# HpWang-whu/YOHO

Hardware: AMD Instinct MI355X
Metric: keypoints/sec (5000 kp x60 rot desc+YOHO-O) (higher is better)
Workload: dtype fp16x2 split (2^-22-accurate products, fp32 accumulate); 1 GPU

## Files before the change

### yoho_amd/csrc/gemmf2.hip

```cpp
#include <hip/hip_runtime.h>
#include <cstdlib>
#include <cstring>
#include "common.h"
#include "gemmf.h"

namespace yoho {

constexpr int F2_BUF = 24576;
constexpr int F2_LDS = 3 * F2_BUF;
constexpr int F3_BUF = 32768;
constexpr int F3_LDS = 3 * F3_BUF;

struct Frags2 {
    uintx4 ah[4], al[4], bh[2], bl[2];
};

template <int LO, int R>
__device__ __forceinline__ void read_frag2(const char* pa, const char* pb, Frags2& f) {
    if constexpr (R < 4) f.al[R] = *reinterpret_cast<const uintx4*>(pa + 8192 + R * 512);
    else if constexpr (R < 6) f.bh[R - 4] = *reinterpret_cast<const uintx4*>(pb + (R - 4) * 512);
    else if constexpr (R < 10) f.ah[R - 6] = *reinterpret_cast<const uintx4*>(pa + (R - 6) * 512);
    else f.bl[R - 10] = *reinterpret_cast<const uintx4*>(pb + LO + (R - 10) * 512);
}
template <int LO>
__device__ __forceinline__ void read_frags2(const char* pa, const char* pb, Frags2& f) {
    sfor<0, 12>([&](auto rc) { read_frag2<LO, decltype(rc)::value>(pa, pb, f); });
}

struct Dma2 {
    static constexpr int NP = 6, LO = 4096;
    int la, lb, w;
    __device__ __forceinline__ Dma2(int w_, int lane) : la(w_ * 1024 + lane * 16), lb((w_ >> 1) * 4096 + (w_ & 1) * 1024 + lane * 16), w(w_) {}
    template <int U>
    __device__ __forceinline__ void piece(const char* srcA, const char* srcB, char* buf) const {
        if constexpr (U < 4) {
            constexpr int plane = U >> 1, kg = U & 1;
            __builtin_amdgcn_global_load_lds((gptr_t)(srcA + plane * 16384 + kg * 4096 + la), (lptr_t)(buf + plane * 8192 + kg * 4096 + w * 1024), 16, 0, 0);
        } else {
            constexpr int plane = U - 4;
            __builtin_amdgcn_global_load_lds((gptr_t)(srcB + plane * 16384 + lb), (lptr_t)(buf + 16384 + plane * 4096 + (w >> 1) * 2048 + (w & 1) * 1024), 16, 0, 0);
        }
    }
};
struct Dma3 {
    static constexpr int NP = 4, LO = 8192;
    int la, ldst;
    __device__ __forceinline__ Dma3(int w8, int lane) : la(w8 * 1024 + lane * 16), ldst(w8 * 1024) {}
    template <int U>
    __device__ __forceinline__ void piece(const char* srcA, const char* srcB, char* buf) const {
        constexpr int plane = U & 1;
        if constexpr (U < 2) __builtin_amdgcn_global_load_lds((gptr_t)(srcA + plane * 16384 + la), (lptr_t)(buf + plane * 8192 + ldst), 16, 0, 0);
        else __builtin_amdgcn_global_load_lds((gptr_t)(srcB + plane * 16384 + la), (lptr_t)(buf + 16384 + plane * 8192 + ldst), 16, 0, 0);
    }
};
template <typename Dma>
__device__ __forceinline__ void dma_step(const Dma& dm, const char* srcA, const char* srcB, char* buf) {
    sfor<0, Dma::NP>([&](auto uc) { dm.template piece<decltype(uc)::value>(srcA, srcB, buf); });
}

template <bool DMA, typename Dma>
__device__ __forceinline__ void step2(const Dma& dm, const Frags2& f, floatx16 (&acc)[4][2], const char* ra, const char* rb, Frags2& nf,
                                      const char* srcA, const char* srcB, char* dmabuf) {
    sfor<0, 8>([&](auto gc) {
        constexpr int g = decltype(gc)::value;
        acc[g >> 1][g & 1] = mfma_h(f.al[g >> 1], f.bh[g & 1], acc[g >> 1][g & 1]);
        read_frag2<Dma::LO, g>(ra, rb, nf);
        __builtin_amdgcn_sched_barrier(0);
    });
    sfor<0, 8>([&](auto gc) {
        constexpr int g = decltype(gc)::value;
        acc[g >> 1][g & 1] = mfma_h(f.ah[g >> 1], f.bl[g & 1], acc[g >> 1][g & 1]);
        if constexpr (g < 4) read_frag2<Dma::LO, 8 + g>(ra, rb, nf);
        else if constexpr (DMA) dm.template piece<g - 4>(srcA, srcB, dmabuf);
        __builtin_amdgcn_sched_barrier(0);
    });
    sfor<0, 8>([&](auto gc) {
        constexpr int g = decltype(gc)::value;
        acc[g >> 1][g & 1] = mfma_h(f.ah[g >> 1], f.bh[g & 1], acc[g >> 1][g & 1]);
        if constexpr (DMA && 4 + g < Dma::NP) dm.template piece<4 + g>(srcA, srcB, dmabuf);
        __builtin_amdgcn_sched_barrier(0);
    });
}

__host__ __device__ inline bool fg2_map(const FGemmArgs& a, int xcd, int slot, bool contiguous, int& t, int& local, int& r) {
    int cnt[NIR_ORD], ru[NIR_ORD];
    for (int u = 0; u < NIR_ORD; ++u) {
        ru[u] = (xcd + a.rot[u]) & 7;
        cnt[u] = a.NT[u] > ru[u] ? ((a.NT[u] - 1 - ru[u]) / 8 + 1) * a.MT[u] * 2 : 0;
    }
    const int L = cnt[0], S = cnt[1] + cnt[2] + cnt[3] + cnt[4];
    int list, idx;
    if (contiguous) { list = slot < L ? 0 : 1; idx = slot < L ? slot : slot - L; }
    else {
        const int P = L < S ? L : S;
        if (slot < 2 * P) { list = slot & 1; idx = slot >> 1; }
        else { list = L > S ? 0 : 1; idx = P + (slot - 2 * P); }
    }
    if (list == 0) {
        if (idx >= L) return false;
        t = 0; local = idx; r = ru[0];
        return true;
    }
    for (int u = 1; u < NIR_ORD; ++u) {
        if (idx < cnt[u]) { t = u; local = idx; r = ru[u]; return true; }
        idx -= cnt[u];
    }
    return false;
}

__device__ __forceinline__ size_t step_off(int ks) { return (size_t)(ks >> 1) * FG_STAGE + (size_t)(ks & 1) * 8192; }

template <int BUF, typename Dma>
__device__ __forceinline__ void ring_prologue(int KT, Dma&& dma) {
    dma(0, 0);
    dma(1, BUF);
    if (KT > 2) dma(2, 2 * BUF);
}

template <int BUF, int INFLIGHT, typename F, typename Step>
__device__ __forceinline__ void ring_pipelined(char* smem, const char* Ag, const char* Bg, int KT, int lane_a, int lane_b, F& P, Step&& step) {
    F Q;
    asm volatile("s_waitcnt lgkmcnt(0)" ::: "memory");
    __builtin_amdgcn_s_barrier();
    __builtin_amdgcn_sched_barrier(0);
    int cur = 0, nxt = BUF;
    int s = 0;
    auto run = [&](auto dma, const F& f, F& nf) {
        if constexpr (decltype(dma)::value) {
            step(dma, f, nf, smem + nxt + lane_a, smem + nxt + lane_b, uniform_ptr(Ag + step_off(s + 3)), uniform_ptr(Bg + step_off(s + 3)), smem + cur);
            asm volatile("s_waitcnt vmcnt(%0) lgkmcnt(0)" ::"n"(INFLIGHT) : "memory");
        } else {
            step(dma, f, nf, smem + nxt + lane_a, smem + nxt + lane_b, nullptr, nullptr, nullptr);
            asm volatile("s_waitcnt vmcnt(0) lgkmcnt(0)" ::: "memory");
        }
        __builtin_amdgcn_s_barrier();
        __builtin_amdgcn_sched_barrier(0);
        cur = nxt; nxt = nxt == 2 * BUF ? 0 : nxt + BUF; ++s;
    };
    constexpr std::true_type dma;
    constexpr std::false_type nodma;
    while (s + 4 < KT) {
        run(dma, P, Q);
        run(dma, Q, P);
    }
    if (KT >= 4) {
        run(dma, P, Q);
        run(nodma, Q, P);
    }
    run(nodma, P, Q);
    step(nodma, Q, P, smem + cur + lane_a, smem + cur + lane_b, nullptr, nullptr, nullptr);
}

template <int BUF, typename Dma>
__device__ __forceinline__ void ring_pipelined_idle(int KT, Dma&& dma) {
    __builtin_amdgcn_s_barrier();
    for (int s = 0; s + 1 < KT; ++s) {
        if (s + 3 < KT) dma(s + 3, (s % 3) * BUF);
        asm volatile("s_waitcnt vmcnt(0)" ::: "memory");
        __builtin_amdgcn_s_barrier();
    }
}

__global__ __launch_bounds__(256, 2) void fgemm2_kernel(FGemmArgs a, int flags) {
    extern __shared__ __attribute__((aligned(16))) char smem[];
    const int tid = threadIdx.x, lane = tid & 63;
    const int w = __builtin_amdgcn_readfirstlane(tid >> 6);
    int t = 0, local = 0, r = 0;
    if (!fg2_map(a, blockIdx.x & 7, blockIdx.x >> 3, (flags & F2_MIX) == 0, t, local, r)) return;
    const int d = a.dim[t];
    const int MT = a.MT[t], KS = d * a.cin / 32, KT = 2 * KS;
    const int nh = local & 1, pair = local >> 1;
    const int cg = pair / MT, mtile = pair - cg * MT;
    const int ntile = r + 8 * cg;
    const char* Ag = a.A + a.a_off[t] + (size_t)mtile * KS * FG_STAGE;
    const char* Bg = a.B + a.b_off[t] + (size_t)ntile * KS * FG_STAGE + nh * 2048;
    const int wm = w >> 1, wn = w & 1;
    const Dma2 dm(w, lane);
    const int lane_a = (lane >> 5) * 4096 + (wm * 128 + (lane & 31)) * 16;
    const int lane_b = 16384 + (lane >> 5) * 2048 + (wn * 64 + (lane & 31)) * 16;

    floatx16 acc[4][2];
    zero_acc(acc);
    auto dma = [&](int st, int buf) { dma_step(dm, Ag + step_off(st), Bg + step_off(st), smem + buf); };
    ring_prologue<F2_BUF>(KT, dma);
    const int row0 = mtile * 256 + wm * 128, colbase = ntile * 256 + nh * 128 + wn * 64;
    const bool rows_live = row0 < d * a.cout;
    const int jidx = colbase / a.kppad, kp0 = colbase - jidx * a.kppad, qbase = a.qbase[t];
    if ((flags & EPI_RES) && rows_live) residual_start(acc, row0, kp0, jidx, d, qbase, a.res, a.descale, a.cout, a.nT32, lane);
    asm volatile("s_waitcnt vmcnt(0)" ::: "memory");
    __builtin_amdgcn_s_barrier();
    if (!rows_live) return ring_pipelined_idle<F2_BUF>(KT, dma);

    Frags2 P;
    read_frags2<Dma2::LO>(smem + lane_a, smem + lane_b, P);
    ring_pipelined<F2_BUF, 6>(smem, Ag, Bg, KT, lane_a, lane_b, P,
        [&](auto dmac, const Frags2& f, Frags2& nf, const char* ra, const char* rb, const char* srcA, const char* srcB, char* buf) {
            step2<decltype(dmac)::value>(dm, f, acc, ra, rb, nf, srcA, srcB, buf);
        });
    coef_epilogue(acc, row0, kp0, jidx, d, qbase, a.out, a.bias, a.descale, a.cout, a.nT32, a.rflag, lane, flags);
}

struct Wave3 {
    int wm, wn, nh, lane_a, lane_b;
    Dma3 dm;
    __device__ __forceinline__ Wave3(int w8, int lane) : wm((w8 & 3) >> 1), wn(w8 & 1), nh(w8 >> 2), dm(w8, lane) {
        lane_a = (lane >> 5) * 4096 + (wm * 128 + (lane & 31)) * 16;
        lane_b = 16384 + (lane >> 5) * 4096 + (nh * 128 + wn * 64 + (lane & 31)) * 16;
    }
};

__global__ __launch_bounds__(512, 2) void fgemm3_kernel(FGemmArgs a, int flags) {
    extern __shared__ __attribute__((aligned(16))) char smem[];
    const int tid = threadIdx.x, lane = tid & 63;
    const Wave3 wv(__builtin_amdgcn_readfirstlane(tid >> 6), lane);
    int t = 0, local = 0, r = 0;
    if (!fg3_map(a, blockIdx.x & 7, blockIdx.x >> 3, t, local, r)) return;
    const int d = a.dim[t];
    const int MT = a.MT[t], KS = d * a.cin / 32, KT = 2 * KS;
    const int cg = local / MT, mtile = local - cg * MT;
    const int ntile = r + 8 * cg;
    const char* Ag = a.A + a.a_off[t] + (size_t)mtile * KS * FG_STAGE;
    const char* Bg = a.B + a.b_off[t] + (size_t)ntile * KS * FG_STAGE;

    floatx16 acc[4][2];
    zero_acc(acc);
    auto dma = [&](int st, int buf) { dma_step(wv.dm, Ag + step_off(st), Bg + step_off(st), smem + buf); };
    ring_prologue<F3_BUF>(KT, dma);
    const int row0 = mtile * 256 + wv.wm * 128, colbase = ntile * 256 + wv.nh * 128 + wv.wn * 64;
    const bool rows_live = row0 < d * a.cout;
    const int jidx = colbase / a.kppad, kp0 = colbase - jidx * a.kppad, qbase = a.qbase[t];
    if ((flags & EPI_RES) && rows_live) residual_start(acc, row0, kp0, jidx, d, qbase, a.res, a.descale, a.cout, a.nT32, lane);
    asm volatile("s_waitcnt vmcnt(0)" ::: "memory");
    __builtin_amdgcn_s_barrier();
    if (!rows_live) return ring_pipelined_idle<F3_BUF>(KT, dma);

    Frags2 P;
    read_frags2<Dma3::LO>(smem + wv.lane_a, smem + wv.lane_b, P);
    ring_pipelined<F3_BUF, 4>(smem, Ag, Bg, KT, wv.lane_a, wv.lane_b, P,
        [&](auto dmac, const Frags2& f, Frags2& nf, const char* ra, const char* rb, const char* srcA, const char* srcB, char* buf) {
            step2<decltype(dmac)::value>(wv.dm, f, acc, ra, rb, nf, srcA, srcB, buf);
        });
    coef_epilogue(acc, row0, kp0, jidx, d, qbase, a.out, a.bias, a.descale, a.cout, a.nT32, a.rflag, lane, flags);
}

constexpr int F3K_BUF = 2 * FG_STAGE;
constexpr int F3K_LDS = 2 * F3K_BUF;

struct Dma3k {
    static constexpr int NP = 8;
    int la, ldst;
    __device__ __forceinline__ Dma3k(int w8, int lane) : la(w8 * 1024 + lane * 16), ldst(w8 * 1024) {}
    template <int U>
    __device__ __forceinline__ void piece(const char* srcA, const char* srcB, char* buf) const {
        constexpr int q = (U & 3) * 8192;
        if constexpr (U < 4) __builtin_amdgcn_global_load_lds((gptr_t)(srcA + q + la), (lptr_t)(buf + q + ldst), 16, 0, 0);
        else __builtin_amdgcn_global_load_lds((gptr_t)(srcB + q + la), (lptr_t)(buf + FG_STAGE + q + ldst), 16, 0, 0);
    }
};
struct FragsA32 { uintx4 al, ah; };
struct FragsB32 { uintx4 bh[4], bl[4]; };

template <int R>
__device__ __forceinline__ void read_open32(const char* pa, const char* pb, FragsA32& a0, FragsB32& b) {
    if constexpr (R == 0) a0.al = *reinterpret_cast<const uintx4*>(pa + 16384);
    else if constexpr (R < 5) b.bh[R - 1] = *reinterpret_cast<const uintx4*>(pb + (R - 1) * 256);
    else if constexpr (R == 5) a0.ah = *reinterpret_cast<const uintx4*>(pa);
    else b.bl[R - 6] = *reinterpret_cast<const uintx4*>(pb + 16384 + (R - 6) * 256);
}

template <bool DMA>
__device__ __forceinline__ void step32(const Dma3k& dm, floatx4 (&acc)[8][4], FragsA32 (&fa)[2], const FragsB32& b, FragsB32& nb, const char* pa,
                                       const char* npa, const char* npb, const char* srcA, const char* srcB, char* dmabuf) {
    sfor<0, 7>([&](auto ic) {
        constexpr int i = decltype(ic)::value;
        row_products32(acc[i], fa[i & 1].al, fa[i & 1].ah, b.bh, b.bl, [&](auto mc) {
            constexpr int m = decltype(mc)::value;
            if constexpr (m == 1) fa[(i + 1) & 1].al = *reinterpret_cast<const uintx4*>(pa + 16384 + (i + 1) * 256);
            if constexpr (m == 2) fa[(i + 1) & 1].ah = *reinterpret_cast<const uintx4*>(pa + (i + 1) * 256);
        });
    });
    asm volatile("s_waitcnt vmcnt(0) lgkmcnt(0)" ::: "memory");
    __builtin_amdgcn_s_barrier();
    __builtin_amdgcn_sched_barrier(0);
    row_products32(acc[7], fa[1].al, fa[1].ah, b.bh, b.bl, [&](auto mc) {
        constexpr int m = decltype(mc)::value;
        if constexpr (m < 5) {
            read_open32<2 * m>(npa, npb, fa[0], nb);
            read_open32<2 * m + 1>(npa, npb, fa[0], nb);
        }
        if constexpr (DMA && m >= 4) dm.template piece<m - 4>(srcA, srcB, dmabuf);
    });
}

__global__ __launch_bounds__(512, 2) void fgemm3k_kernel(FGemmArgs a, int flags) {
    extern __shared__ __attribute__((aligned(16))) char smem[];
    const int tid = threadIdx.x, lane = tid & 63;
    const int w8 = __builtin_amdgcn_readfirstlane(tid >> 6);
    int t = 0, local = 0, r = 0;
    if (!fg3_map(a, blockIdx.x & 7, blockIdx.x >> 3, t, local, r)) return;
    const int d = a.dim[t];
    const int MT = a.MT[t], KS = d * a.cin / 32;
    const int cg = local / MT, mtile = local - cg * MT;
    const int ntile = r + 8 * cg;
    const char* Ag = a.A + a.a_off[t] + (size_t)mtile * KS * FG_STAGE;
    const char* Bg = a.B + a.b_off[t] + (size_t)ntile * KS * FG_STAGE;
    const int wm = (w8 & 3) >> 1, wn = w8 & 1, nh = w8 >> 2;
    const Dma3k dm(w8, lane);
    const int lane_a = (lane >> 4) * 4096 + (wm * 128 + (lane & 15)) * 16;
    const int lane_b = FG_STAGE + (lane >> 4) * 4096 + (nh * 128 + wn * 64 + (lane & 15)) * 16;

    floatx4 acc[8][4];
    zero_acc(acc);
    auto dma = [&](int st, int buf) {
        const char* sa = uniform_ptr(Ag + (size_t)st * FG_STAGE);
        const char* sb = uniform_ptr(Bg + (size_t)st * FG_STAGE);
        sfor<0, Dma3k::NP>([&](auto uc) { dm.template piece<decltype(uc)::value>(sa, sb, smem + buf); });
    };
    dma(0, 0);
    if (KS > 1) dma(1, F3K_BUF);
    const int row0 = mtile * 256 + wm * 128, colbase = ntile * 256 + nh * 128 + wn * 64;
    const bool rows_live = row0 < d * a.cout;
    const int jidx = colbase / a.kppad, kp0 = colbase - jidx * a.kppad, qbase = a.qbase[t];
    if ((flags & EPI_RES) && rows_live) residual_start(acc, row0, kp0, jidx, d, qbase, a.res, a.descale, a.cout, a.nT32, lane);
    asm volatile("s_waitcnt vmcnt(0)" ::: "memory");
    __builtin_amdgcn_s_barrier();
    if (!rows_live) {
        for (int s = 0; s < KS; ++s) {
            asm volatile("s_waitcnt vmcnt(0)" ::: "memory");
            __builtin_amdgcn_s_barrier();
            if (s + 2 < KS) dma(s + 2, (s & 1) * F3K_BUF);
        }
        asm volatile("s_waitcnt vmcnt(0)" ::: "memory");
        return;
    }

    FragsA32 fa[2];
    FragsB32 P, Q;
    sfor<0, 10>([&](auto rc) { read_open32<decltype(rc)::value>(smem + lane_a, smem + lane_b, fa[0], P); });
    int s = 0, cur = 0;
    auto run = [&](auto dmac, const FragsB32& b, FragsB32& nb) {
        const int nxt = cur ^ F3K_BUF;
        if constexpr (decltype(dmac)::value)
            step32<true>(dm, acc, fa, b, nb, smem + cur + lane_a, smem + nxt + lane_a, smem + nxt + lane_b, uniform_ptr(Ag + (size_t)(s + 2) * FG_STAGE),
                         uniform_ptr(Bg + (size_t)(s + 2) * FG_STAGE), smem + cur);
        else
            step32<false>(dm, acc, fa, b, nb, smem + cur + lane_a, smem + nxt + lane_a, smem + nxt + lane_b, nullptr, nullptr, nullptr);
        cur = nxt; ++s;
    };
    constexpr std::true_type dmay;
    constexpr std::false_type dman;
    while (s + 2 < KS) {
        run(dmay, P, Q);
        run(dmay, Q, P);
    }
    run(dman, P, Q);
    run(dman, Q, P);
    coef_epilogue(acc, row0, kp0, jidx, d, qbase, a.out, a.bias, a.descale, a.cout, a.nT32, a.rflag, lane, flags);
}

constexpr int F2K_BUF = FG_STAGE + FG_STAGE / 2;
constexpr int F2K_LDS = 2 * F2K_BUF;

__global__ __launch_bounds__(256, 1) void fgemm2k_kernel(FGemmArgs a, int flags) {
    extern __shared__ __attribute__((aligned(16))) char smem[];
    const int tid = threadIdx.x, lane = tid & 63;
    const int w = __builtin_amdgcn_readfirstlane(tid >> 6);
    int t = 0, local = 0, r = 0;
    if (!fg2_map(a, blockIdx.x & 7, blockIdx.x >> 3, (flags & F2_MIX) == 0, t, local, r)) return;
    const int d = a.dim[t];
    const int MT = a.MT[t], KS = d * a.cin / 32;
    const int nh = local & 1, pair = local >> 1;
    const int cg = pair / MT, mtile = pair - cg * MT;
    const int ntile = r + 8 * cg;
    const char* Ag = a.A + a.a_off[t] + (size_t)mtile * KS * FG_STAGE;
    const char* Bg = a.B + a.b_off[t] + (size_t)ntile * KS * FG_STAGE + nh * 2048;
    const int wm = w >> 1, wn = w & 1;
    const int lane_a = (lane >> 4) * 4096 + (wm * 128 + (lane & 15)) * 16;
    const int lane_b = FG_STAGE + (lane >> 4) * 2048 + (wn * 64 + (lane & 15)) * 16;

    floatx4 acc[8][4];
    zero_acc(acc);
    auto dma = [&](int st, int buf) {
        const char* sa = uniform_ptr(Ag + (size_t)st * FG_STAGE) + lane * 16;
        const char* sb = uniform_ptr(Bg + (size_t)st * FG_STAGE) + lane * 16;
#pragma unroll
        for (int k = 0; k < 8; ++k) __builtin_amdgcn_global_load_lds((gptr_t)(sa + (k * 4 + w) * 1024), (lptr_t)(smem + buf + (k * 4 + w) * 1024), 16, 0, 0);
#pragma unroll
        for (int k = 0; k < 4; ++k) {
            const int pb = w * 4 + k, u = pb >> 1, part = pb & 1;
            __builtin_amdgcn_global_load_lds((gptr_t)(sb + u * 4096 + part * 1024), (lptr_t)(smem + buf + FG_STAGE + u * 2048 + part * 1024), 16, 0, 0);
        }
    };
    dma(0, 0);
    if (KS > 1) dma(1, F2K_BUF);
    const int row0 = mtile * 256 + wm * 128, colbase = ntile * 256 + nh * 128 + wn * 64;
    const bool rows_live = row0 < d * a.cout;
    const int jidx = colbase / a.kppad, kp0 = colbase - jidx * a.kppad, qbase = a.qbase[t];
    if ((flags & EPI_RES) && rows_live) residual_start(acc, row0, kp0, jidx, d, qbase, a.res, a.descale, a.cout, a.nT32, lane);
    asm volatile("s_waitcnt vmcnt(0)" ::: "memory");
    __builtin_amdgcn_s_barrier();
    for (int s = 0; s < KS; ++s) {
        const int cur = (s & 1) * F2K_BUF;
        if (rows_live) stage32_plain<FG_STAGE / 4>(acc, smem + cur + lane_a, smem + cur + lane_b);
        asm volatile("s_waitcnt vmcnt(0) lgkmcnt(0)" ::: "memory");
        __builtin_amdgcn_s_barrier();
        __builtin_amdgcn_sched_barrier(0);
        if (s + 2 < KS) dma(s + 2, cur);
    }
    if (rows_live) coef_epilogue(acc, row0, kp0, jidx, d, qbase, a.out, a.bias, a.descale, a.cout, a.nT32, a.rflag, lane, flags);
}

typedef int intx8 __attribute__((ext_vector_type(8)));
typedef short shortx2 __attribute__((ext_vector_type(2)));
typedef _Float16 halfx2 __attribute__((ext_vector_type(2)));
struct Frags8 {
    intx8 a[4], b[2];
};
struct C8Scales {
    float ah = 4.f, al = 4.f / 2048.f, bh = 1.f, bl = 1.f;
    int mfma_b = 127;
    C8Scales() = default;
    __device__ __forceinline__ explicit C8Scales(const unsigned* amax) {
        const unsigned amax_bits = __builtin_amdgcn_readfirstlane(*amax);
        int kexp = (int)(amax_bits >> 23) - 127 - 7;
        kexp = kexp < -60 ? -60 : (kexp > 9 ? 9 : kexp);
        bh = __uint_as_float((unsigned)(kexp + 127) << 23); bl = __uint_as_float((unsigned)(kexp - 11 + 127) << 23);
        mfma_b = 127 + kexp;
    }
};
struct Int2 { int x, y; };
__device__ __forceinline__ Int2 frag_to_fp8(uintx4 f, float scale) {
    union { unsigned u; halfx2 h; } p0, p1, p2, p3;
    p0.u = f[0]; p1.u = f[1]; p2.u = f[2]; p3.u = f[3];
    shortx2 r = {0, 0}, q = {0, 0};
    r = __builtin_amdgcn_cvt_scalef32_pk_fp8_f16(r, p0.h, scale, false);
    r = __builtin_amdgcn_cvt_scalef32_pk_fp8_f16(r, p1.h, scale, true);
    q = __builtin_amdgcn_cvt_scalef32_pk_fp8_f16(q, p2.h, scale, false);
    q = __builtin_amdgcn_cvt_scalef32_pk_fp8_f16(q, p3.h, scale, true);
    Int2 o;
    __builtin_memcpy(&o.x, &r, 4);
    __builtin_memcpy(&o.y, &q, 4);
    return o;
}

template <int PAR>
__device__ __forceinline__ void step3c(const Frags2& f, floatx16 (&acc)[4][2], Frags8& c8, const C8Scales& sc) {
#pragma unroll
    for (int i = 0; i < 4; ++i)
#pragma unroll
        for (int j = 0; j < 2; ++j) acc[i][j] = mfma_h(f.ah[i], f.bh[j], acc[i][j]);
#pragma unroll
    for (int i = 0; i < 4; ++i)
#pragma unroll
        for (int e = 0; e < 4; ++e) c8.a[i][4 * PAR + e] = (int)f.al[i][e];
#pragma unroll
    for (int j = 0; j < 2; ++j) {
        const Int2 l = frag_to_fp8(f.bl[j], sc.bl), h = frag_to_fp8(f.bh[j], sc.bh);
        c8.b[j][4 * PAR] = l.x; c8.b[j][4 * PAR + 1] = l.y; c8.b[j][4 * PAR + 2] = h.x; c8.b[j][4 * PAR + 3] = h.y;
    }
    if constexpr (PAR == 1) {
#pragma unroll
        for (int i = 0; i < 4; ++i)
#pragma unroll
            for (int j = 0; j < 2; ++j)
                acc[i][j] = __builtin_amdgcn_mfma_scale_f32_32x32x64_f8f6f4(c8.a[i], c8.b[j], acc[i][j], 0, 0, 0, 127 + 2 - 11, 0, sc.mfma_b);
    }
}

template <bool FP8, typename BSrc>
__device__ __forceinline__ void ring_plain(floatx16 (&acc)[4][2], char* smem, const Wave3& wv, const char* Ag, BSrc&& bsrc, int KT, bool rows_live,
                                           const C8Scales& sc) {
    Frags8 c8;
    if constexpr (FP8) {
#pragma unroll
        for (int i = 0; i < 4; ++i)
#pragma unroll
            for (int e = 0; e < 8; ++e) c8.a[i][e] = 0;
#pragma unroll
        for (int j = 0; j < 2; ++j)
#pragma unroll
            for (int e = 0; e < 8; ++e) c8.b[j][e] = 0;
    }
    int cur = 0, stg = 2 * F3_BUF;
    int s = 0;
    auto stage = [&] {
        const int s2 = s + 2 < KT ? s + 2 : KT - 1;
        dma_step(wv.dm, uniform_ptr(Ag + step_off(s2)), uniform_ptr(bsrc(s2)), smem + stg);
    };
    auto rotate = [&] { stg = cur; cur = cur == 2 * F3_BUF ? 0 : cur + F3_BUF; ++s; };
    auto one_step = [&](auto parity) {
        asm volatile("s_waitcnt vmcnt(4) lgkmcnt(0)" ::: "memory");
        __builtin_amdgcn_s_barrier();
        __builtin_amdgcn_sched_barrier(0);
        stage();
        Frags2 f;
        read_frags2<Dma3::LO>(smem + cur + wv.lane_a, smem + cur + wv.lane_b, f);
        if constexpr (FP8) step3c<decltype(parity)::value>(f, acc, c8, sc);
        else {
#pragma unroll
            for (int i = 0; i < 4; ++i)
#pragma unroll
                for (int j = 0; j < 2; ++j) acc[i][j] = mfma_h(f.al[i], f.bh[j], acc[i][j]);
#pragma unroll
            for (int i = 0; i < 4; ++i)
#pragma unroll
                for (int j = 0; j < 2; ++j) acc[i][j] = mfma_h(f.ah[i], f.bl[j], acc[i][j]);
#pragma unroll
            for (int i = 0; i < 4; ++i)
#pragma unroll
                for (int j = 0; j < 2; ++j) acc[i][j] = mfma_h(f.ah[i], f.bh[j], acc[i][j]);
        }
        rotate();
    };
    if (rows_live) {
        for (int it = 0; it < KT; it += 2) {
            one_step(std::integral_constant<int, 0>{});
            one_step(std::integral_constant<int, 1>{});
        }
    } else {
        for (int it = 0; it < KT; ++it) {
            asm volatile("s_waitcnt vmcnt(4) lgkmcnt(0)" ::: "memory");
            __builtin_amdgcn_s_barrier();
            stage();
            rotate();
        }
    }
    asm volatile("s_waitcnt vmcnt(0)" ::: "memory");
}

__global__ __launch_bounds__(512, 2) void fgemm3c_kernel(FGemmArgs a, int flags) {
    extern __shared__ __attribute__((aligned(16))) char smem[];
    const int tid = threadIdx.x, lane = tid & 63;
    const Wave3 wv(__builtin_amdgcn_readfirstlane(tid >> 6), lane);
    int t = 0, local = 0, r = 0;
    if (!fg3_map(a, blockIdx.x & 7, blockIdx.x >> 3, t, local, r)) return;
    const int d = a.dim[t];
    const int MT = a.MT[t], KS = d * a.cin / 32, KT = 2 * KS;
    const int cg = local / MT, mtile = local - cg * MT;
    const int ntile = r + 8 * cg;
    const char* Ag = a.A + a.a_off[t] + (size_t)mtile * KS * FG_STAGE;
    const char* Bg = a.B + a.b_off[t] + (size_t)ntile * KS * FG_STAGE;

    floatx16 acc[4][2];
    zero_acc(acc);
    const C8Scales sc(a.amax);
    dma_step(wv.dm, Ag, Bg, smem);
    dma_step(wv.dm, Ag + step_off(1), Bg + step_off(1), smem + F3_BUF);
    const int row0 = mtile * 256 + wv.wm * 128, colbase = ntile * 256 + wv.nh * 128 + wv.wn * 64;
    const bool rows_live = row0 < d * a.cout;
    const int jidx = colbase / a.kppad, kp0 = colbase - jidx * a.kppad, qbase = a.qbase[t];
    if ((flags & EPI_RES) && rows_live) residual_start(acc, row0, kp0, jidx, d, qbase, a.res, a.descale, a.cout, a.nT32, lane);
    asm volatile("s_waitcnt vmcnt(0)" ::: "memory");
    __builtin_amdgcn_s_barrier();

    ring_plain<true>(acc, smem, wv, Ag, [&](int s) { return Bg + step_off(s); }, KT, rows_live, sc);
    if (rows_live) coef_epilogue(acc, row0, kp0, jidx, d, qbase, a.out, a.bias, a.descale, a.cout, a.nT32, a.rflag, lane, flags);
}

struct CGemmArgs {
    const char* A;
    const char* B;
    const float* bias;
    const float* bn_s;
    const float* bn_t;
    char* out;
    int NTm, MT, KSt, ntap, nj, nslot, c8out, nT32, nTiles16;
    float descale;
    int* rflag;
    const unsigned* amax;
    unsigned char slot[13 * 13];
    unsigned char outg[16];
};

__device__ __forceinline__ void cg_split_pair(float x0, float x1, unsigned& hi, unsigned& lo) {
    typedef float f2 __attribute__((ext_vector_type(2)));
    f2 x;
    x.x = x0; x.y = x1;
    const halfx2 h = __builtin_convertvector(x, halfx2);
    const f2 r = x - __builtin_convertvector(h, f2);
    const halfx2 l = __builtin_convertvector(r, halfx2);
    __builtin_memcpy(&hi, &h, 4);
    __builtin_memcpy(&lo, &l, 4);
}

template <bool FP8>
__global__ __launch_bounds__(512, 2) void cgemm_kernel(CGemmArgs a) {
    extern __shared__ __attribute__((aligned(16))) char smem[];
    __shared__ int tapoff[16];
    const int tid = threadIdx.x, lane = tid & 63;
    const Wave3 wv(__builtin_amdgcn_readfirstlane(tid >> 6), lane);
    const int xcd = blockIdx.x & 7, slot_ = blockIdx.x >> 3;
    const int ct = xcd + 8 * (slot_ / a.MT), mtile = slot_ % a.MT;
    if (ct >= a.nj * a.NTm) return;
    const int j = ct / a.NTm, mt = ct - j * a.NTm;
    const int SPT = 2 * a.KSt;
    const int KT = a.ntap * SPT;
    if (tid < 16) tapoff[tid] = tid < a.ntap ? (int)a.slot[j * 13 + tid] : 0;
    const char* Ag = a.A + (size_t)mtile * (KT / 2) * FG_STAGE;
    const char* Bt = a.B + (size_t)mt * a.nslot * a.KSt * FG_STAGE;
    __syncthreads();
    auto bsrc = [&](int s) -> const char* {
        const int tap = s / SPT, within = s - tap * SPT;
        const int sl = __builtin_amdgcn_readfirstlane(tapoff[tap]);
        return Bt + (size_t)sl * a.KSt * FG_STAGE + step_off(within);
    };

    floatx16 acc[4][2];
    zero_acc(acc);
    C8Scales sc;
    if constexpr (FP8) sc = C8Scales(a.amax);
    dma_step(wv.dm, Ag, uniform_ptr(bsrc(0)), smem);
    dma_step(wv.dm, Ag + step_off(1), uniform_ptr(bsrc(1)), smem + F3_BUF);
    asm volatile("s_waitcnt vmcnt(0)" ::: "memory");
    __builtin_amdgcn_s_barrier();

    ring_plain<FP8>(acc, smem, wv, Ag, bsrc, KT, true, sc);

    const int half = lane >> 5, c32 = lane & 31;
    const int g = a.outg[j];
    unsigned top = 0u;
#pragma unroll
    for (int bi = 0; bi < 2; ++bi) {
        const int m = mt * 256 + wv.nh * 128 + wv.wn * 64 + bi * 32 + c32;
        if ((m >> 5) >= a.nT32 || (m >> 4) >= a.nTiles16) continue;
#pragma unroll
        for (int ai = 0; ai < 4; ++ai) {
#pragma unroll
            for (int q4 = 0; q4 < 4; ++q4) {
                const int o = mtile * 256 + wv.wm * 128 + ai * 32 + q4 * 8 + half * 4;
                const floatx4 b4 = *reinterpret_cast<const floatx4*>(a.bias + o);
                const floatx4 s4 = *reinterpret_cast<const floatx4*>(a.bn_s + o);
                const floatx4 t4 = *reinterpret_cast<const floatx4*>(a.bn_t + o);
                float y[4];
#pragma unroll
                for (int e = 0; e < 4; ++e) {
                    const float v = acc[ai][bi][4 * q4 + e] * a.descale + b4[e];
                    y[e] = fmaxf(v * s4[e] + t4[e], 0.f) * H2_ASCALE;
                    top = max(top, __float_as_uint(y[e]) & 0x7FFFFFFFu);
                }
                unsigned h0, l0, h1, l1;
                cg_split_pair(y[0], y[1], h0, l0);
                cg_split_pair(y[2], y[3], h1, l1);
                char* dst = a.out + (((size_t)(m >> 4) * a.c8out + (o >> 3)) * 2) * 15360 + g * 256 + (m & 15) * 16 + half * 8;
                *reinterpret_cast<uint2*>(dst) = uint2{h0, h1};
                *reinterpret_cast<uint2*>(dst + 15360) = uint2{l0, l1};
            }
        }
    }
    note_range_bits(a.rflag, top, FP16_MAX);
}

__global__ __launch_bounds__(512, 2) void cgemmk_kernel(CGemmArgs a) {
    extern __shared__ __attribute__((aligned(16))) char smem[];
    __shared__ int tapoff[16];
    const int tid = threadIdx.x, lane = tid & 63;
    const int w8 = __builtin_amdgcn_readfirstlane(tid >> 6);
    const int xcd = blockIdx.x & 7, slot_ = blockIdx.x >> 3;
    const int ct = xcd + 8 * (slot_ / a.MT), mtile = slot_ % a.MT;
    if (ct >= a.nj * a.NTm) return;
    const int j = ct / a.NTm, mt = ct - j * a.NTm;
    const int KS = a.ntap * a.KSt;
    if (tid < 16) tapoff[tid] = tid < a.ntap ? (int)a.slot[j * 13 + tid] : 0;
    const char* Ag = a.A + (size_t)mtile * KS * FG_STAGE;
    const char* Bt = a.B + (size_t)mt * a.nslot * a.KSt * FG_STAGE;
    __syncthreads();
    auto bsrc = [&](int st) -> const char* {
        const int tap = st / a.KSt, cb = st - tap * a.KSt;
        const int sl = __builtin_amdgcn_readfirstlane(tapoff[tap]);
        return uniform_ptr(Bt + ((size_t)sl * a.KSt + cb) * FG_STAGE);
    };
    const int wm = (w8 & 3) >> 1, wn = w8 & 1, nh = w8 >> 2;
    const Dma3k dm(w8, lane);
    const int lane_a = (lane >> 4) * 4096 + (wm * 128 + (lane & 15)) * 16;
    const int lane_b = FG_STAGE + (lane >> 4) * 4096 + (nh * 128 + wn * 64 + (lane & 15)) * 16;

    floatx4 acc[8][4];
    zero_acc(acc);
    auto dma = [&](int st, int buf) {
        const char* sa = uniform_ptr(Ag + (size_t)st * FG_STAGE);
        const char* sb = bsrc(st);
        sfor<0, Dma3k::NP>([&](auto uc) { dm.template piece<decltype(uc)::value>(sa, sb, smem + buf); });
    };
    dma(0, 0);
    dma(1, F3K_BUF);
    asm volatile("s_waitcnt vmcnt(0)" ::: "memory");
    __builtin_amdgcn_s_barrier();

    FragsA32 fa[2];
    FragsB32 P, Q;
    sfor<0, 10>([&](auto rc) { read_open32<decltype(rc)::value>(smem + lane_a, smem + lane_b, fa[0], P); });
    int s = 0, cur = 0;
    auto run = [&](auto dmac, const FragsB32& b, FragsB32& nb) {
        const int nxt = cur ^ F3K_BUF;
        if constexpr (decltype(dmac)::value)
            step32<true>(dm, acc, fa, b, nb, smem + cur + lane_a, smem + nxt + lane_a, smem + nxt + lane_b, uniform_ptr(Ag + (size_t)(s + 2) * FG_STAGE),
                         bsrc(s + 2), smem + cur);
        else
            step32<false>(dm, acc, fa, b, nb, smem + cur + lane_a, smem + nxt + lane_a, smem + nxt + lane_b, nullptr, nullptr, nullptr);
        cur = nxt; ++s;
    };
    constexpr std::true_type dmay;
    constexpr std::false_type dman;
    while (s + 2 < KS) {
        run(dmay, P, Q);
        run(dmay, Q, P);
    }
    run(dman, P, Q);
    run(dman, Q, P);

    int etid = threadIdx.x;
    asm volatile("" : "+v"(etid));
    const int g4 = (etid >> 4) & 3, c16 = etid & 15;
    const int g = a.outg[j];
    const int col0 = mt * 256 + nh * 128 + wn * 64;
    unsigned top = 0u;
#pragma unroll
    for (int ai = 0; ai < 8; ++ai) {
        const int o = mtile * 256 + wm * 128 + ai * 16 + g4 * 4;
        const floatx4 b4 = *reinterpret_cast<const floatx4*>(a.bias + o);
        const floatx4 s4 = *reinterpret_cast<const floatx4*>(a.bn_s + o);
        const floatx4 t4 = *reinterpret_cast<const floatx4*>(a.bn_t + o);
#pragma unroll
        for (int bi = 0; bi < 4; ++bi) {
            const int m0 = col0 + bi * 16;
            if ((m0 >> 5) >= a.nT32 || (m0 >> 4) >= a.nTiles16) continue;
            float y[4];
#pragma unroll
            for (int e = 0; e < 4; ++e) {
                const float v = acc[ai][bi][e] * a.descale + b4[e];
                y[e] = fmaxf(v * s4[e] + t4[e], 0.f) * H2_ASCALE;
                top = max(top, __float_as_uint(y[e]) & 0x7FFFFFFFu);
            }
            unsigned h0, l0, h1, l1;
            cg_split_pair(y[0], y[1], h0, l0);
            cg_split_pair(y[2], y[3], h1, l1);
            char* dst = a.out + (((size_t)(m0 >> 4) * a.c8out + (o >> 3)) * 2) * 15360 + g * 256 + c16 * 16 + (g4 & 1) * 8;
            *reinterpret_cast<uint2*>(dst) = uint2{h0, h1};
            *reinterpret_cast<uint2*>(dst + 15360) = uint2{l0, l1};
        }
    }
    note_range_bits(a.rflag, top, FP16_MAX);
}

int cgemm_init() {
    HIPCHK(hipFuncSetAttribute(reinterpret_cast<const void*>(&cgemm_kernel<true>), hipFuncAttributeMaxDynamicSharedMemorySize, F3_LDS));
    HIPCHK(hipFuncSetAttribute(reinterpret_cast<const void*>(&cgemm_kernel<false>), hipFuncAttributeMaxDynamicSharedMemorySize, F3_LDS));
    HIPCHK(hipFuncSetAttribute(reinterpret_cast<const void*>(&cgemmk_kernel), hipFuncAttributeMaxDynamicSharedMemorySize, F3K_LDS));
    return 0;
}

int launch_cgemm(const Layer& L, const char* Bstages, int nslot, const unsigned char* slot, const unsigned char* outg, int nT32, int nTiles16,
                 char* out, hipStream_t s, int* rflag, const unsigned* amax) {
    const bool fp8 = amax != nullptr;
    if (!(fp8 ? L.wcg8 : L.wcg) || L.cin % 32 || L.cout % 256) { set_error("cgemm: needs the cone-GEMM weight pack, cin %% 32 == 0, cout %% 256 == 0"); return YOHO_EINVAL; }
    if (nT32 == 0) return 0;
    CGemmArgs a;
    a.A = reinterpret_cast<const char*>(fp8 ? L.wcg8 : L.wcg); a.B = Bstages; a.bias = L.bias; a.bn_s = L.bn_s; a.bn_t = L.bn_t; a.out = out;
    a.NTm = (nT32 + 7) / 8; a.MT = L.cout / 256; a.KSt = L.cin / 32; a.ntap = 13; a.nj = 13; a.nslot = nslot; a.c8out = L.cout / 8;
    a.nT32 = nT32; a.nTiles16 = nTiles16; a.descale = L.wcg_descale; a.rflag = rflag; a.amax = amax;
    std::memcpy(a.slot, slot, 169);
    std::memset(a.outg, 0, 16);
    std::memcpy(a.outg, outg, 13);
    const int CT = a.nj * a.NTm;
    const int grid = 8 * ((CT + 7) / 8) * a.MT;
    const char* dbg = experiment_env("YOHO_FGEMM_DEBUG");
    const bool k32 = !fp8 && (a.ntap * a.KSt) % 2 == 0 && !(dbg && std::strstr(dbg, "k16"));
    if (fp8) hipLaunchKernelGGL(cgemm_kernel<true>, dim3(grid), dim3(512), F3_LDS, s, a);
    else if (k32) hipLaunchKernelGGL(cgemmk_kernel, dim3(grid), dim3(512), F3K_LDS, s, a);
    else hipLaunchKernelGGL(cgemm_kernel<false>, dim3(grid), dim3(512), F3_LDS, s, a);
    HIPCHK(hipGetLastError());
    return 0;
}

struct Frags3s {
    uintx4 ah[5], al[5], bh, bl;
};

template <int R>
__device__ __forceinline__ void read_frag3s(const char* pa, const char* pb, Frags3s& f) {
    if constexpr (R < 5) f.al[R] = *reinterpret_cast<const uintx4*>(pa + 8192 + R * 512);
    else if constexpr (R == 5) f.bh = *reinterpret_cast<const uintx4*>(pb);
    else if constexpr (R < 11) f.ah[R - 6] = *reinterpret_cast<const uintx4*>(pa + (R - 6) * 512);
    else f.bl = *reinterpret_cast<const uintx4*>(pb + 8192);
}

template <bool DMA, int D>
__device__ __forceinline__ void step3s(const Frags3s& f, floatx16 (&acc)[5][1], const char* ra, const char* rb, Frags3s& nf,
                                       const char* srcA, const char* srcB, char* dmabuf, const Dma3& dm) {
    sfor<0, 5>([&](auto gc) {
        constexpr int g = decltype(gc)::value;
        if constexpr (g < D) acc[g][0] = mfma_h(f.al[g], f.bh, acc[g][0]);
        if constexpr (g < D) read_frag3s<g>(ra, rb, nf);
        if constexpr (g == 4) read_frag3s<5>(ra, rb, nf);
        __builtin_amdgcn_sched_barrier(0);
    });
    sfor<0, 5>([&](auto gc) {
        constexpr int g = decltype(gc)::value;
        if constexpr (g < D) acc[g][0] = mfma_h(f.ah[g], f.bl, acc[g][0]);
        if constexpr (g < D) read_frag3s<6 + g>(ra, rb, nf);
        if constexpr (g == 4) read_frag3s<11>(ra, rb, nf);
        __builtin_amdgcn_sched_barrier(0);
    });
    sfor<0, 5>([&](auto gc) {
        constexpr int g = decltype(gc)::value;
        if constexpr (g < D) acc[g][0] = mfma_h(f.ah[g], f.bh, acc[g][0]);
        if constexpr (DMA && g < 4) dm.template piece<g>(srcA, srcB, dmabuf);
        __builtin_amdgcn_sched_barrier(0);
    });
}

template <int D>
__device__ __forceinline__ void fgemm3s_kloop(floatx16 (&acc)[5][1], char* smem, const char* Ag, const char* Bg, int KT, const Dma3& dm, int lane_a, int lane_b) {
    Frags3s P;
    sfor<0, 12>([&](auto rc) {
        constexpr int R = decltype(rc)::value;
        if constexpr (R == 5 || R == 11 || (R < 5 && R < D) || (R > 5 && R < 11 && R - 6 < D)) read_frag3s<R>(smem + lane_a, smem + lane_b, P);
    });
    ring_pipelined<F3_BUF, 4>(smem, Ag, Bg, KT, lane_a, lane_b, P,
        [&](auto dmac, const Frags3s& f, Frags3s& nf, const char* ra, const char* rb, const char* srcA, const char* srcB, char* buf) {
            step3s<decltype(dmac)::value, D>(f, acc, ra, rb, nf, srcA, srcB, buf, dm);
        });
}

__global__ __launch_bounds__(512, 2) void fgemm3s_kernel(FGemmArgs a, int flags) {
    extern __shared__ __attribute__((aligned(16))) char smem[];
    const int tid = threadIdx.x, lane = tid & 63;
    const int w8 = __builtin_amdgcn_readfirstlane(tid >> 6);
    int t = 0, local = 0, r = 0;
    if (!fg3_map(a, blockIdx.x & 7, blockIdx.x >> 3, t, local, r)) return;
    const int d = a.dim[t];
    const int KS = d * a.cin / 32, KT = 2 * KS;
    const int ntile = r + 8 * local;
    const char* Ag = a.A + a.a_off[t];
    const char* Bg = a.B + a.b_off[t] + (size_t)ntile * KS * FG_STAGE;
    const Dma3 dm(w8, lane);
    const int lane_a = (lane >> 5) * 4096 + (lane & 31) * 16;
    const int lane_b = 16384 + (lane >> 5) * 4096 + (w8 * 32 + (lane & 31)) * 16;

    floatx16 acc[5][1];
    zero_acc(acc);
    ring_prologue<F3_BUF>(KT, [&](int st, int buf) { dma_step(dm, uniform_ptr(Ag + step_off(st)), uniform_ptr(Bg + step_off(st)), smem + buf); });
    asm volatile("s_waitcnt vmcnt(0)" ::: "memory");
    __builtin_amdgcn_s_barrier();

    switch (d) {
        case 1: fgemm3s_kloop<1>(acc, smem, Ag, Bg, KT, dm, lane_a, lane_b); break;
        case 3: fgemm3s_kloop<3>(acc, smem, Ag, Bg, KT, dm, lane_a, lane_b); break;
        case 4: fgemm3s_kloop<4>(acc, smem, Ag, Bg, KT, dm, lane_a, lane_b); break;
        default: fgemm3s_kloop<5>(acc, smem, Ag, Bg, KT, dm, lane_a, lane_b); break;
    }
    const int colbase = ntile * 256 + w8 * 32;
    const int jidx = colbase / a.kppad, kp0 = colbase - jidx * a.kppad;
    coef_epilogue(acc, 0, kp0, jidx, d, a.qbase[t], a.out, a.bias, a.descale, 32, a.nT32, a.rflag, lane, flags & F2_NOSTORE);
}

int fgemm3_init() {
    HIPCHK(hipFuncSetAttribute(reinterpret_cast<const void*>(&fgemm3_kernel), hipFuncAttributeMaxDynamicSharedMemorySize, F3_LDS));
    HIPCHK(hipFuncSetAttribute(reinterpret_cast<const void*>(&fgemm3s_kernel), hipFuncAttributeMaxDynamicSharedMemorySize, F3_LDS));
    HIPCHK(hipFuncSetAttribute(reinterpret_cast<const void*>(&fgemm3c_kernel), hipFuncAttributeMaxDynamicSharedMemorySize, F3_LDS));
    HIPCHK(hipFuncSetAttribute(reinterpret_cast<const void*>(&fgemm3k_kernel), hipFuncAttributeMaxDynamicSharedMemorySize, F3K_LDS));
    return 0;
}

int launch_fgemm3(const FGemmArgs& a, int flags, hipStream_t s) {
    if (const char* dbg = experiment_env("YOHO_FGEMM_DEBUG")) {
        if (std::strstr(dbg, "nostore")) flags |= F2_NOSTORE;
        if (std::strstr(dbg, "sc1")) flags |= F2_ST_SC1;
        if (std::strstr(dbg, "stnt")) flags |= F2_ST_NT;
    }
    const int tot = fgemm_grid(a, 1);
    static const bool small_ok = [] { const char* e = experiment_env("YOHO_FGEMM_DEBUG"); return !(e && std::strstr(e, "nosmall")); }();
    if (small_ok && a.cout == 32 && !(flags & EPI_RES)) hipLaunchKernelGGL(fgemm3s_kernel, dim3(tot), dim3(512), F3_LDS, s, a, flags);
    else if (a.amax) hipLaunchKernelGGL(fgemm3c_kernel, dim3(tot), dim3(512), F3_LDS, s, a, flags);
    else if (flags & F2_K32) hipLaunchKernelGGL(fgemm3k_kernel, dim3(tot), dim3(512), F3K_LDS, s, a, flags);
    else hipLaunchKernelGGL(fgemm3_kernel, dim3(tot), dim3(512), F3_LDS, s, a, flags);
    HIPCHK(hipGetLastError());
    return 0;
}

int fgemm2_init() {
    HIPCHK(hipFuncSetAttribute(reinterpret_cast<const void*>(&fgemm2_kernel), hipFuncAttributeMaxDynamicSharedMemorySize, F2_LDS));
    HIPCHK(hipFuncSetAttribute(reinterpret_cast<const void*>(&fgemm2k_kernel), hipFuncAttributeMaxDynamicSharedMemorySize, F2K_LDS));
    return fgemm3_init();
}

int launch_fgemm2(const FGemmArgs& a, int flags, hipStream_t s) {
    if (const char* dbg = experiment_env("YOHO_FGEMM_DEBUG")) {
        if (std::strstr(dbg, "nostore")) flags |= F2_NOSTORE;
        if (std::strstr(dbg, "mix")) flags |= F2_MIX;
        if (std::strstr(dbg, "sc1")) flags |= F2_ST_SC1;
        if (std::strstr(dbg, "nt")) flags |= F2_ST_NT;
        if (std::strstr(dbg, "sparse4")) flags |= F2_SPARSE4;
        if (std::strstr(dbg, "sparse16")) flags |= F2_SPARSE16;
    }
    if (flags & F2_K32) hipLaunchKernelGGL(fgemm2k_kernel, dim3(fgemm_grid(a, 2)), dim3(256), F2K_LDS, s, a, flags);
    else hipLaunchKernelGGL(fgemm2_kernel, dim3(fgemm_grid(a, 2)), dim3(256), F2_LDS, s, a, flags);
    HIPCHK(hipGetLastError());
    return 0;
}

}
```

Before: 1.961 million keypoints/s.

## Add deep five-buffer ring with dimension-sized stages for cout=32 fgemm3 kernel

Adds a new small-output fgemm3 kernel that uses a 5-deep LDS ring, with buffer size scaled to the rotation dimension d instead of a fixed 32KB. Only the A rows that are needed are DMA'd, per-piece offsets are precomputed, and the waits are counted rather than draining. The B loads use an aux cache-policy bit (AUX=2). It is selected when cout==32 and cin is large enough; the old 3-buffer kernel is kept as a fallback. The aim is to hide global load latency and cut wasted transfers. The cost is more LDS per block and more complex synchronisation.

```diff
diff --git a/yoho_amd/csrc/gemmf2.hip b/yoho_amd/csrc/gemmf2.hip
--- a/yoho_amd/csrc/gemmf2.hip
+++ b/yoho_amd/csrc/gemmf2.hip
@@ -822,7 +822,7 @@
         });
 }
 
-__global__ __launch_bounds__(512, 2) void fgemm3s_kernel(FGemmArgs a, int flags) {
+__global__ __launch_bounds__(512, 2) void fgemm3s_ring3_kernel(FGemmArgs a, int flags) {
     extern __shared__ __attribute__((aligned(16))) char smem[];
     const int tid = threadIdx.x, lane = tid & 63;
     const int w8 = __builtin_amdgcn_readfirstlane(tid >> 6);
@@ -854,9 +854,171 @@
     coef_epilogue(acc, 0, kp0, jidx, d, a.qbase[t], a.out, a.bias, a.descale, 32, a.nT32, a.rflag, lane, flags & F2_NOSTORE);
 }
 
+constexpr int F3S_NB = 5;
+constexpr int F3S_AUX = 2;
+#ifdef YOHO_EXPERIMENTS
+constexpr int F3S_AUX_ALT = 0;
+#endif
+constexpr int f3s_buf(int d) { return 16384 + 2048 * d; }
+constexpr int F3S_LDS = F3S_NB * f3s_buf(5);
+
+template <int D, int AUX>
+struct Dma3s {
+    static constexpr int NAW = (2 * D) / 8, NAX = (2 * D) % 8, NPW = 2 + NAW;
+    int lb, ldst, aoff[NAW + 1];
+    bool extra;
+    __device__ __forceinline__ Dma3s(int w8, int lane) : lb(w8 * 1024 + lane * 16), ldst(w8 * 1024), extra(w8 < NAX) {
+#pragma unroll
+        for (int i = 0; i <= NAW; ++i) {
+            const int c = min((w8 + 8 * i) * 64 + lane, 128 * D - 1);
+            const int b = c / (32 * D), r = c - b * (32 * D);
+            aoff[i] = (b >> 1) * 16384 + (b & 1) * 4096 + r * 16;
+        }
+    }
+    template <int U>
+    __device__ __forceinline__ void piece(const char* srcA, const char* srcB, char* buf) const {
+        if constexpr (U < 2) __builtin_amdgcn_global_load_lds((gptr_t)(srcB + U * 16384 + lb), (lptr_t)(buf + U * 8192 + ldst), 16, 0, AUX);
+        else __builtin_amdgcn_global_load_lds((gptr_t)(srcA + aoff[U - 2]), (lptr_t)(buf + 16384 + (U - 2) * 8192 + ldst), 16, 0, 0);
+    }
+    __device__ __forceinline__ void step(const char* srcA, const char* srcB, char* buf) const {
+        sfor<0, NPW>([&](auto uc) { piece<decltype(uc)::value>(srcA, srcB, buf); });
+        if constexpr (NAX > 0) if (extra) piece<NPW>(srcA, srcB, buf);
+    }
+    template <int STEPS>
+    __device__ __forceinline__ void wait() const {
+        if (NAX > 0 && STEPS > 0 && extra) asm volatile("s_waitcnt vmcnt(%0) lgkmcnt(0)" ::"n"(STEPS * (NPW + 1)) : "memory");
+        else asm volatile("s_waitcnt vmcnt(%0) lgkmcnt(0)" ::"n"(STEPS * NPW) : "memory");
+    }
+};
+
+template <int D, int R>
+__device__ __forceinline__ void read_frag3d(const char* pa, const char* pb, Frags3s& f) {
+    if constexpr (R < 5) f.al[R] = *reinterpret_cast<const uintx4*>(pa + 1024 * D + R * 512);
+    else if constexpr (R == 5) f.bh = *reinterpret_cast<const uintx4*>(pb);
+    else if constexpr (R < 11) f.ah[R - 6] = *reinterpret_cast<const uintx4*>(pa + (R - 6) * 512);
+    else f.bl = *reinterpret_cast<const uintx4*>(pb + 8192);
+}
+
+template <bool DMA, int D, int AUX>
+__device__ __forceinline__ void step3d(const Frags3s& f, floatx16 (&acc)[5][1], const char* ra, const char* rb, Frags3s& nf,
+                                       const char* srcA, const char* srcB, char* dmabuf, const Dma3s<D, AUX>& dm) {
+    using Dm = Dma3s<D, AUX>;
+    sfor<0, 5>([&](auto gc) {
+        constexpr int g = decltype(gc)::value;
+        if constexpr (g < D) acc[g][0] = mfma_h(f.al[g], f.bh, acc[g][0]);
+        if constexpr (g < D) read_frag3d<D, g>(ra, rb, nf);
+        if constexpr (g == 4) read_frag3d<D, 5>(ra, rb, nf);
+        __builtin_amdgcn_sched_barrier(0);
+    });
+    sfor<0, 5>([&](auto gc) {
+        constexpr int g = decltype(gc)::value;
+        if constexpr (g < D) acc[g][0] = mfma_h(f.ah[g], f.bl, acc[g][0]);
+        if constexpr (g < D) read_frag3d<D, 6 + g>(ra, rb, nf);
+        if constexpr (g == 4) read_frag3d<D, 11>(ra, rb, nf);
+        __builtin_amdgcn_sched_barrier(0);
+    });
+    sfor<0, 5>([&](auto gc) {
+        constexpr int g = decltype(gc)::value;
+        if constexpr (g < D) acc[g][0] = mfma_h(f.ah[g], f.bh, acc[g][0]);
+        if constexpr (DMA && g < Dm::NPW) dm.template piece<g>(srcA, srcB, dmabuf);
+        if constexpr (DMA && g == Dm::NPW && Dm::NAX > 0) if (dm.extra) dm.template piece<g>(srcA, srcB, dmabuf);
+        __builtin_amdgcn_sched_barrier(0);
+    });
+}
+
+template <int D, int NB, int AUX>
+__device__ __forceinline__ void fgemm3s_deep(floatx16 (&acc)[5][1], char* smem, const char* Ag, const char* Bg, int KT, int w, int lane) {
+    using Dm = Dma3s<D, AUX>;
+    static_assert(NB >= 3 && (NB - 2) * (Dm::NPW + 1) < 64 && Dm::NPW < 5, "the counted wait must fit vmcnt, the pieces the third product row");
+    constexpr int BUF = f3s_buf(D);
+    const Dm dm(w, lane);
+    const int lane_a = 16384 + (lane >> 5) * 512 * D + (lane & 31) * 16;
+    const int lane_b = (lane >> 5) * 4096 + (w * 32 + (lane & 31)) * 16;
+    sfor<0, NB>([&](auto sc) {
+        constexpr int st = decltype(sc)::value;
+        dm.step(uniform_ptr(Ag + step_off(st)), uniform_ptr(Bg + step_off(st)), smem + st * BUF);
+    });
+    dm.template wait<NB - 2>();
+    __builtin_amdgcn_s_barrier();
+    Frags3s P, Q;
+    sfor<0, 12>([&](auto rc) {
+        constexpr int R = decltype(rc)::value;
+        if constexpr (R == 5 || R == 11 || (R < 5 && R < D) || (R > 5 && R < 11 && R - 6 < D)) read_frag3d<D, R>(smem + lane_a, smem + lane_b, P);
+    });
+    asm volatile("s_waitcnt lgkmcnt(0)" ::: "memory");
+    __builtin_amdgcn_s_barrier();
+    __builtin_amdgcn_sched_barrier(0);
+    int cur = 0, nxt = BUF;
+    int s = 0;
+    auto advance = [&] {
+        __builtin_amdgcn_s_barrier();
+        __builtin_amdgcn_sched_barrier(0);
+        cur = nxt; nxt = nxt == (NB - 1) * BUF ? 0 : nxt + BUF; ++s;
+    };
+    auto run_dma = [&](const Frags3s& f, Frags3s& nf) {
+        step3d<true, D, AUX>(f, acc, smem + nxt + lane_a, smem + nxt + lane_b, nf, uniform_ptr(Ag + step_off(s + NB)), uniform_ptr(Bg + step_off(s + NB)), smem + cur, dm);
+        dm.template wait<NB - 2>();
+        advance();
+    };
+    while (s + NB + 1 < KT) {
+        run_dma(P, Q);
+        run_dma(Q, P);
+    }
+    auto tail = [&](Frags3s& f, Frags3s& nf) {
+        sfor<0, NB>([&](auto ic) {
+            constexpr int i = decltype(ic)::value;
+            const Frags3s& a = (i & 1) ? nf : f;
+            Frags3s& b = (i & 1) ? f : nf;
+            if constexpr (i + 1 < NB) {
+                step3d<false, D, AUX>(a, acc, smem + nxt + lane_a, smem + nxt + lane_b, b, nullptr, nullptr, nullptr, dm);
+                dm.template wait<(NB - 3 - i > 0 ? NB - 3 - i : 0)>();
+                advance();
+            } else {
+                step3d<false, D, AUX>(a, acc, smem + cur + lane_a, smem + cur + lane_b, b, nullptr, nullptr, nullptr, dm);
+            }
+        });
+    };
+    if constexpr (NB & 1) {
+        run_dma(P, Q);
+        tail(Q, P);
+    } else {
+        tail(P, Q);
+    }
+}
+
+template <int NB, int AUX>
+__global__ __launch_bounds__(512, 2) void fgemm3s_kernel(FGemmArgs a, int flags) {
+    extern __shared__ __attribute__((aligned(16))) char smem[];
+    const int tid = threadIdx.x, lane = tid & 63;
+    const int w8 = __builtin_amdgcn_readfirstlane(tid >> 6);
+    int t = 0, local = 0, r = 0;
+    if (!fg3_map(a, blockIdx.x & 7, blockIdx.x >> 3, t, local, r)) return;
+    const int d = a.dim[t];
+    const int KS = d * a.cin / 32, KT = 2 * KS;
+    const int ntile = r + 8 * local;
+    const char* Ag = a.A + a.a_off[t];
+    const char* Bg = a.B + a.b_off[t] + (size_t)ntile * KS * FG_STAGE;
+
+    floatx16 acc[5][1];
+    zero_acc(acc);
+    switch (d) {
+        case 1: fgemm3s_deep<1, NB, AUX>(acc, smem, Ag, Bg, KT, w8, lane); break;
+        case 3: fgemm3s_deep<3, NB, AUX>(acc, smem, Ag, Bg, KT, w8, lane); break;
+        case 4: fgemm3s_deep<4, NB, AUX>(acc, smem, Ag, Bg, KT, w8, lane); break;
+        default: fgemm3s_deep<5, NB, AUX>(acc, smem, Ag, Bg, KT, w8, lane); break;
+    }
+    const int colbase = ntile * 256 + w8 * 32;
+    const int jidx = colbase / a.kppad, kp0 = colbase - jidx * a.kppad;
+    coef_epilogue(acc, 0, kp0, jidx, d, a.qbase[t], a.out, a.bias, a.descale, 32, a.nT32, a.rflag, lane, flags & F2_NOSTORE);
+}
+
 int fgemm3_init() {
     HIPCHK(hipFuncSetAttribute(reinterpret_cast<const void*>(&fgemm3_kernel), hipFuncAttributeMaxDynamicSharedMemorySize, F3_LDS));
-    HIPCHK(hipFuncSetAttribute(reinterpret_cast<const void*>(&fgemm3s_kernel), hipFuncAttributeMaxDynamicSharedMemorySize, F3_LDS));
+    HIPCHK(hipFuncSetAttribute(reinterpret_cast<const void*>(&fgemm3s_ring3_kernel), hipFuncAttributeMaxDynamicSharedMemorySize, F3_LDS));
+    HIPCHK(hipFuncSetAttribute(reinterpret_cast<const void*>(&fgemm3s_kernel<F3S_NB, F3S_AUX>), hipFuncAttributeMaxDynamicSharedMemorySize, F3S_LDS));
+#ifdef YOHO_EXPERIMENTS
+    HIPCHK(hipFuncSetAttribute(reinterpret_cast<const void*>(&fgemm3s_kernel<F3S_NB, F3S_AUX_ALT>), hipFuncAttributeMaxDynamicSharedMemorySize, F3S_LDS));
+#endif
     HIPCHK(hipFuncSetAttribute(reinterpret_cast<const void*>(&fgemm3c_kernel), hipFuncAttributeMaxDynamicSharedMemorySize, F3_LDS));
     HIPCHK(hipFuncSetAttribute(reinterpret_cast<const void*>(&fgemm3k_kernel), hipFuncAttributeMaxDynamicSharedMemorySize, F3K_LDS));
     return 0;
@@ -870,7 +1032,15 @@
     }
     const int tot = fgemm_grid(a, 1);
     static const bool small_ok = [] { const char* e = experiment_env("YOHO_FGEMM_DEBUG"); return !(e && std::strstr(e, "nosmall")); }();
-    if (small_ok && a.cout == 32 && !(flags & EPI_RES)) hipLaunchKernelGGL(fgemm3s_kernel, dim3(tot), dim3(512), F3_LDS, s, a, flags);
+    const char* dbg = experiment_env("YOHO_FGEMM_DEBUG");
+    const bool small = small_ok && a.cout == 32 && !(flags & EPI_RES);
+    const bool deep = small && a.cin / 16 >= 2 * F3S_NB && !(dbg && std::strstr(dbg, "s3ring"));
+#ifdef YOHO_EXPERIMENTS
+    if (deep && dbg && std::strstr(dbg, "s3alt")) hipLaunchKernelGGL((fgemm3s_kernel<F3S_NB, F3S_AUX_ALT>), dim3(tot), dim3(512), F3S_LDS, s, a, flags);
+    else
+#endif
+    if (deep) hipLaunchKernelGGL((fgemm3s_kernel<F3S_NB, F3S_AUX>), dim3(tot), dim3(512), F3S_LDS, s, a, flags);
+    else if (small) hipLaunchKernelGGL(fgemm3s_ring3_kernel, dim3(tot), dim3(512), F3_LDS, s, a, flags);
     else if (a.amax) hipLaunchKernelGGL(fgemm3c_kernel, dim3(tot), dim3(512), F3_LDS, s, a, flags);
     else if (flags & F2_K32) hipLaunchKernelGGL(fgemm3k_kernel, dim3(tot), dim3(512), F3K_LDS, s, a, flags);
     else hipLaunchKernelGGL(fgemm3_kernel, dim3(tot), dim3(512), F3_LDS, s, a, flags);
```

Measured after the change: 1.967 million keypoints/s (median of 6 runs). About the same (+0.3%).
